# Hawkeye-FineGrained/Hawkeye

Measured on NVIDIA H100. Metric: 448x448 images/sec, BCNN VGG-16 train step (fwd+CE+bwd+grad all-reduce+SGD), device-timed, max over ranks, higher is better.
Workload: dtype tf32 (fp32 storage, fp32 accumulate)

## Files before the change

### hawkeye_b200/csrc/conv.cu

```cuda
#include <stdlib.h>

#include "common.cuh"
#include "host.h"
#include "gemm.h"
#include "../../include/hawkeye_b200.h"

namespace hk {

__global__ void pack_weights_kernel(const float* __restrict__ W, float* __restrict__ Wf, float* __restrict__ Wd,
                                    int Cout, int Cin, int round) {
  const size_t n = (size_t)Cout * Cin * 9;
  for (size_t i = blockIdx.x * (size_t)blockDim.x + threadIdx.x; i < n; i += (size_t)gridDim.x * blockDim.x) {
    const int t = i % 9;
    const int ci = (i / 9) % Cin;
    const int co = i / ((size_t)9 * Cin);
    const float v = round ? tf32_round(W[i]) : W[i];
    if (Wf) Wf[((size_t)t * Cout + co) * Cin + ci] = v;
    if (Wd) Wd[((size_t)(8 - t) * Cin + ci) * Cout + co] = v;
  }
}
__global__ void unpack_wgrad_kernel(const float* __restrict__ dWp, float* __restrict__ dW, int Cout, int Cin, int accumulate) {
  const size_t n = (size_t)Cout * Cin * 9;
  for (size_t i = blockIdx.x * (size_t)blockDim.x + threadIdx.x; i < n; i += (size_t)gridDim.x * blockDim.x) {
    const int t = i % 9;
// ... 813 lines not shown
  a.total_tiles = (int)total_tiles;
  a.per = (int)((total_tiles + ks - 1) / ks);
  const dim3 grid((unsigned)out_tiles, (unsigned)((total_tiles + a.per - 1) / a.per));
  CUtensorMap tmDY, tmX;
  int r;
  if ((r = make_act_map(&tmDY, dy, a.N, a.H, a.W, a.Cout, a.TW, a.TH, a.TN))) return r;
  if ((r = make_act_map(&tmX, x, a.N, a.H, a.W, a.Cin, a.TW + 2, a.TH + 2, a.TN))) return r;
  if (a.TW == 16 && a.TH == 4 && a.TN == 1) return launch_wgrad_tile<16, 4, 1>(tmDY, tmX, a, grid, stream);
  if (a.TW == 8 && a.TH == 8 && a.TN == 1) return launch_wgrad_tile<8, 8, 1>(tmDY, tmX, a, grid, stream);
  if (a.TW == 8 && a.TH == 4 && a.TN == 2) return launch_wgrad_tile<8, 4, 2>(tmDY, tmX, a, grid, stream);
  return set_error(HK_ERR_UNSUPPORTED, "conv3x3_wgrad: pixel tile %dx%dx%d has no kernel", a.TW, a.TH, a.TN);
}

static int conv3x3_wgrad_1x(const float* x, const float* dy, float* dwp, float* db, int N, int H, int W, int Cin, int Cout,
                            cudaStream_t stream, bool zero_dw, bool zero_db);

int conv3x3_wgrad(const float* x, const float* dy, float* dwp, float* db, int N, int H, int W, int Cin, int Cout,
                  cudaStream_t stream, bool zero_db = true) {
  if (!precise()) return conv3x3_wgrad_1x(x, dy, dwp, db, N, H, W, Cin, Cout, stream, true, zero_db);
  HK_REQUIRE(x && dy && dwp, HK_ERR_ARG, "conv3x3_wgrad: null pointer");
  const size_t nx = (size_t)N * H * W * Cin, ny = (size_t)N * H * W * Cout;
  Scratch sx(2 * nx * sizeof(float), stream), sy(2 * ny * sizeof(float), stream);
  HK_REQUIRE(sx.p && sy.p, HK_ERR_DRIVER, "conv3x3_wgrad (precise): cudaMallocAsync of the operand halves failed");
  float *xh = sx.f(), *xl = xh + nx, *yh = sy.f(), *yl = yh + ny;
  int r;
  if ((r = tf32_split(x, xh, xl, nx, stream))) return r;
  if ((r = tf32_split(dy, yh, yl, ny, stream))) return r;
  if ((r = conv3x3_wgrad_1x(xh, yh, dwp, db, N, H, W, Cin, Cout, stream, true, zero_db))) return r;
  if ((r = conv3x3_wgrad_1x(xl, yh, dwp, nullptr, N, H, W, Cin, Cout, stream, false, false))) return r;
  return conv3x3_wgrad_1x(xh, yl, dwp, db, N, H, W, Cin, Cout, stream, false, false);
}

static int conv3x3_wgrad_1x(const float* x, const float* dy, float* dwp, float* db, int N, int H, int W, int Cin, int Cout,
                            cudaStream_t stream, bool zero_dw, bool zero_db) {
  HK_REQUIRE(x && dy && dwp, HK_ERR_ARG, "conv3x3_wgrad: null pointer");
  HK_REQUIRE(Cin % 32 == 0 && Cout % 32 == 0, HK_ERR_UNSUPPORTED, "conv3x3_wgrad: Cin=%d Cout=%d unsupported", Cin, Cout);
  WgradArgs a = {};
  a.dWp = dwp; a.db = db; a.N = N; a.H = H; a.W = W; a.Cin = Cin; a.Cout = Cout;
  pick_wgrad_tile(W, H, &a.TW, &a.TH, &a.TN);
  HK_REQUIRE((a.TH + 2) * (a.TW + 2) * a.TN <= WG_RAW_ROWS, HK_ERR_UNSUPPORTED,
             "conv3x3_wgrad: halo patch too large");
  a.tiles_w = (W + a.TW - 1) / a.TW; a.tiles_h = (H + a.TH - 1) / a.TH; a.tiles_n = (N + a.TN - 1) / a.TN;
  cudaError_t e = cudaSuccess;
  if (zero_dw) {
    e = cudaMemsetAsync(dwp, 0, (size_t)9 * Cout * Cin * sizeof(float), stream);
    if (e != cudaSuccess) return set_error((int)e, "cudaMemsetAsync(dWp): %s", cudaGetErrorString(e));
  }
  if (db && zero_db) {
    e = cudaMemsetAsync(db, 0, (size_t)Cout * sizeof(float), stream);
    if (e != cudaSuccess) return set_error((int)e, "cudaMemsetAsync(db): %s", cudaGetErrorString(e));
  }
  return launch_wgrad(x, dy, a, stream);
}

__global__ void im2col_first_kernel(const float* __restrict__ x, float* __restrict__ x27, int N, int H, int W, int round) {
  const long long total = (long long)N * H * W;
  for (long long pix = blockIdx.x * (long long)blockDim.x + threadIdx.x; pix < total;
       pix += (long long)gridDim.x * blockDim.x) {
    const int wq = (int)(pix % W), hq = (int)((pix / W) % H), n = (int)(pix / ((long long)W * H));
    float v[32];
#pragma unroll
    for (int ci = 0; ci < 3; ++ci)
#pragma unroll
      for (int kh = 0; kh < 3; ++kh)
#pragma unroll
        for (int kw = 0; kw < 3; ++kw) {
          const int hh = hq + kh - 1, ww = wq + kw - 1;
          float t = (hh >= 0 && hh < H && ww >= 0 && ww < W) ? __ldg(x + (((size_t)n * 3 + ci) * H + hh) * W + ww) : 0.f;
          v[ci * 9 + kh * 3 + kw] = round ? tf32_round(t) : t;
        }
    v[27] = 1.f; v[28] = v[29] = v[30] = v[31] = 0.f;
    float4* dst = reinterpret_cast<float4*>(x27 + (size_t)pix * 32);
#pragma unroll
    for (int j = 0; j < 8; ++j) dst[j] = make_float4(v[4 * j], v[4 * j + 1], v[4 * j + 2], v[4 * j + 3]);
  }
}
__global__ void pack_first_weights_kernel(const float* __restrict__ w, const float* __restrict__ bias,
                                          float* __restrict__ w27, int Cout, int round) {
  const int i = blockIdx.x * blockDim.x + threadIdx.x;
  if (i >= Cout * 32) return;
  const int co = i / 32, r = i % 32;
  const float t = r < 27 ? w[co * 27 + r] : (r == 27 && bias ? bias[co] : 0.f);
  w27[i] = round ? tf32_round(t) : t;
}

__global__ void maxpool2x2_fwd_kernel(const float* __restrict__ x, float* __restrict__ y, int N, int H, int W, int C,
                                      int out_nchw) {
  const int Ho = H / 2, Wo = W / 2, C4 = C / 4;
  const size_t total = (size_t)N * Ho * Wo * C4;
  for (size_t i = blockIdx.x * (size_t)blockDim.x + threadIdx.x; i < total; i += (size_t)gridDim.x * blockDim.x) {
    const int c4 = i % C4;
    size_t p = i / C4;
    const int wo = p % Wo; p /= Wo;
    const int ho = p % Ho;
    const int n = p / Ho;
    const float4* base = reinterpret_cast<const float4*>(x + (((size_t)n * H + 2 * ho) * W + 2 * wo) * C) + c4;
    const float4 a = base[0], b = base[C4], c = base[(size_t)W * C4], d = base[(size_t)W * C4 + C4];
    float4 m;
    m.x = fmaxf(fmaxf(a.x, b.x), fmaxf(c.x, d.x));
    m.y = fmaxf(fmaxf(a.y, b.y), fmaxf(c.y, d.y));
    m.z = fmaxf(fmaxf(a.z, b.z), fmaxf(c.z, d.z));
    m.w = fmaxf(fmaxf(a.w, b.w), fmaxf(c.w, d.w));
    if (!out_nchw) {
      reinterpret_cast<float4*>(y + (((size_t)n * Ho + ho) * Wo + wo) * C)[c4] = m;
    } else {
      const size_t hw = (size_t)Ho * Wo, o = ((size_t)n * C + c4 * 4) * hw + (size_t)ho * Wo + wo;
      y[o] = m.x; y[o + hw] = m.y; y[o + 2 * hw] = m.z; y[o + 3 * hw] = m.w;
    }
  }
}

__global__ void maxpool2x2_bwd_kernel(const float* __restrict__ x, const float* __restrict__ dy,
                                      float* __restrict__ dx, int N, int H, int W, int C, int dy_nchw) {
  const int Ho = H / 2, Wo = W / 2;
  const size_t total = (size_t)N * Ho * Wo * C;
  for (size_t i = blockIdx.x * (size_t)blockDim.x + threadIdx.x; i < total; i += (size_t)gridDim.x * blockDim.x) {
    const int c = i % C;
    size_t p = i / C;
    const int wo = p % Wo; p /= Wo;
    const int ho = p % Ho;
    const int n = p / Ho;
    const size_t b00 = (((size_t)n * H + 2 * ho) * W + 2 * wo) * C + c;
    const size_t b01 = b00 + C, b10 = b00 + (size_t)W * C, b11 = b10 + C;
    const float v00 = x[b00], v01 = x[b01], v10 = x[b10], v11 = x[b11];
    const float g = dy_nchw ? dy[((size_t)n * C + c) * Ho * Wo + (size_t)ho * Wo + wo] : dy[i];
    int arg = 0;
    float m = v00;
    if (v01 > m) { m = v01; arg = 1; }
    if (v10 > m) { m = v10; arg = 2; }
    if (v11 > m) { m = v11; arg = 3; }
    const float gm = m > 0.f ? g : 0.f;
    dx[b00] = arg == 0 ? gm : 0.f;
    dx[b01] = arg == 1 ? gm : 0.f;
    dx[b10] = arg == 2 ? gm : 0.f;
    dx[b11] = arg == 3 ? gm : 0.f;
  }
}

__global__ void maxpool2x2_fwd_idx_kernel(const float* __restrict__ x, float* __restrict__ y, unsigned char* __restrict__ code,
                                          int N, int H, int W, int C, int out_nchw) {
  const int Ho = H / 2, Wo = W / 2, C4 = C / 4;
  const size_t total = (size_t)N * Ho * Wo * C4;
  for (size_t i = blockIdx.x * (size_t)blockDim.x + threadIdx.x; i < total; i += (size_t)gridDim.x * blockDim.x) {
    const int c4 = i % C4;
    size_t p = i / C4;
    const int wo = p % Wo; p /= Wo;
    const int ho = p % Ho;
    const int n = p / Ho;
    const float4* base = reinterpret_cast<const float4*>(x + (((size_t)n * H + 2 * ho) * W + 2 * wo) * C) + c4;
    const float4 v0 = base[0], v1 = base[C4], v2 = base[(size_t)W * C4], v3 = base[(size_t)W * C4 + C4];
    float4 m = v0;
    uchar4 a = make_uchar4(0, 0, 0, 0);
#define HK_POOL_STEP(V, K)                     \
    if (V.x > m.x) { m.x = V.x; a.x = K; }     \
    if (V.y > m.y) { m.y = V.y; a.y = K; }     \
    if (V.z > m.z) { m.z = V.z; a.z = K; }     \
    if (V.w > m.w) { m.w = V.w; a.w = K; }
    HK_POOL_STEP(v1, 1) HK_POOL_STEP(v2, 2) HK_POOL_STEP(v3, 3)
#undef HK_POOL_STEP
    a.x |= m.x > 0.f ? 4 : 0; a.y |= m.y > 0.f ? 4 : 0; a.z |= m.z > 0.f ? 4 : 0; a.w |= m.w > 0.f ? 4 : 0;
    reinterpret_cast<uchar4*>(code)[i] = a;
    if (!out_nchw) {
      reinterpret_cast<float4*>(y + (((size_t)n * Ho + ho) * Wo + wo) * C)[c4] = m;
    } else {
      const size_t hw = (size_t)Ho * Wo, o = ((size_t)n * C + c4 * 4) * hw + (size_t)ho * Wo + wo;
      y[o] = m.x; y[o + hw] = m.y; y[o + 2 * hw] = m.z; y[o + 3 * hw] = m.w;
// ... 79 lines not shown
int hk_conv3x3_dgrad(const float* dy, const float* w_dgrad_packed, const float* relu_mask_act, float* dx, int N, int H,
                     int W, int Cin, int Cout, void* stream) {
  return conv3x3_igemm(dy, w_dgrad_packed, nullptr, relu_mask_act, dx, N, H, W, Cout, Cin, 0, (cudaStream_t)stream);
}

size_t hk_conv3x3_wgrad_workspace_bytes(int Cin, int Cout) { return (size_t)9 * Cin * Cout * sizeof(float); }

int hk_conv3x3_wgrad_acc(const float* x, const float* dy, float* dw, float* db, int N, int H, int W, int Cin, int Cout,
                         void* workspace, size_t workspace_bytes, int accumulate, void* stream_) {
  cudaStream_t stream = (cudaStream_t)stream_;
  HK_REQUIRE(workspace && workspace_bytes >= hk_conv3x3_wgrad_workspace_bytes(Cin, Cout), HK_ERR_WORKSPACE,
             "hk_conv3x3_wgrad: workspace too small");
  HK_REQUIRE(dw, HK_ERR_ARG, "hk_conv3x3_wgrad: null dw");
  float* dwp = static_cast<float*>(workspace);
  int r = conv3x3_wgrad(x, dy, dwp, db, N, H, W, Cin, Cout, stream, !accumulate);
  if (r) return r;
  unpack_wgrad_kernel<<<grid_1d((size_t)Cout * Cin * 9, 256), 256, 0, stream>>>(dwp, dw, Cout, Cin, accumulate ? 1 : 0);
  HK_LAUNCH_CHECK("unpack_wgrad_kernel");
  return 0;
}

int hk_conv3x3_wgrad(const float* x, const float* dy, float* dw, float* db, int N, int H, int W, int Cin, int Cout,
                     void* workspace, size_t workspace_bytes, void* stream_) {
  return hk_conv3x3_wgrad_acc(x, dy, dw, db, N, H, W, Cin, Cout, workspace, workspace_bytes, 0, stream_);
}

size_t hk_conv3x3_first_fwd_workspace_bytes(int N, int H, int W, int Cout) {
  return ((size_t)N * H * W * 32 + (size_t)Cout * 32) * sizeof(float);
}

int hk_conv3x3_first_fwd(const float* x_nchw, const float* w, const float* bias, float* y_nhwc, int N, int H, int W,
                         int Cout, void* workspace, size_t workspace_bytes, void* stream_) {
  cudaStream_t stream = (cudaStream_t)stream_;
  HK_REQUIRE(x_nchw && w && y_nhwc, HK_ERR_ARG, "hk_conv3x3_first_fwd: null pointer");
  HK_REQUIRE(Cout % 4 == 0 && Cout <= 256, HK_ERR_UNSUPPORTED, "hk_conv3x3_first_fwd: Cout=%d unsupported", Cout);
  HK_REQUIRE(workspace && workspace_bytes >= hk_conv3x3_first_fwd_workspace_bytes(N, H, W, Cout), HK_ERR_WORKSPACE,
             "hk_conv3x3_first_fwd: workspace too small");
  const long long P = (long long)N * H * W;
  HK_REQUIRE(P < (1ll << 31), HK_ERR_UNSUPPORTED, "hk_conv3x3_first_fwd: too many pixels");
  float* x27 = static_cast<float*>(workspace);
  float* w27 = x27 + (size_t)P * 32;
  const int round = precise() ? 0 : 1;
  im2col_first_kernel<<<grid_1d((size_t)P, 128), 128, 0, stream>>>(x_nchw, x27, N, H, W, round);
  HK_LAUNCH_CHECK("im2col_first_kernel");
  pack_first_weights_kernel<<<(Cout * 32 + 127) / 128, 128, 0, stream>>>(w, bias, w27, Cout, round);
  HK_LAUNCH_CHECK("pack_first_weights_kernel");
  GemmEpi e = {};
  e.C = y_nhwc; e.ldc = Cout; e.alpha = 1.f;
  e.relu = 3;
  return gemm_tf32(x27, 0, 32, 0, w27, 0, 32, 0, e, (int)P, Cout, 32, 1, stream);
}

static int first_wgrad_splits(long long P) {
  for (int S = 592; S > 1; --S)
    if (P % S == 0) return S;
  return 1;
}

size_t hk_conv3x3_first_wgrad_workspace_bytes(int N, int H, int W, int Cout) {
  return (size_t)first_wgrad_splits((long long)N * H * W) * Cout * 32 * sizeof(float);
}

int hk_conv3x3_first_wgrad_acc(const float* x27, const float* dy_nhwc, float* dw, float* db, int N, int H, int W, int Cout,
                               void* workspace, size_t workspace_bytes, int accumulate, void* stream_);
int hk_conv3x3_first_wgrad(const float* x27, const float* dy_nhwc, float* dw, float* db, int N, int H, int W,
                           int Cout, void* workspace, size_t workspace_bytes, void* stream_) {
  return hk_conv3x3_first_wgrad_acc(x27, dy_nhwc, dw, db, N, H, W, Cout, workspace, workspace_bytes, 0, stream_);
}
int hk_conv3x3_first_wgrad_acc(const float* x27, const float* dy_nhwc, float* dw, float* db, int N, int H, int W, int Cout,
                               void* workspace, size_t workspace_bytes, int accumulate, void* stream_) {
  cudaStream_t stream = (cudaStream_t)stream_;
  HK_REQUIRE(x27 && dy_nhwc && dw, HK_ERR_ARG, "hk_conv3x3_first_wgrad: null pointer");
  HK_REQUIRE(Cout % 4 == 0 && Cout <= 128, HK_ERR_UNSUPPORTED, "hk_conv3x3_first_wgrad: Cout=%d unsupported", Cout);
  HK_REQUIRE(workspace && workspace_bytes >= hk_conv3x3_first_wgrad_workspace_bytes(N, H, W, Cout), HK_ERR_WORKSPACE,
             "hk_conv3x3_first_wgrad: workspace too small");
  const long long P = (long long)N * H * W;
  const int S = first_wgrad_splits(P);
  float* part = static_cast<float*>(workspace);
  int r = gemm_splitk(dy_nhwc, 1, Cout, x27, 1, 32, Cout, 32, P, S, part, dw, 27, 27, nullptr, accumulate, stream);
  if (r || !db) return r;
  return sum_splits(part + 27, S, (long long)Cout * 32, Cout, 1, 32, db, 1, nullptr, accumulate, stream);
}

int hk_maxpool2x2_fwd(const float* x_nhwc, float* y, int N, int H, int W, int C, int out_nchw, void* stream) {
  HK_REQUIRE(x_nhwc && y, HK_ERR_ARG, "hk_maxpool2x2_fwd: null pointer");
  HK_REQUIRE(C % 4 == 0 && H % 2 == 0 && W % 2 == 0, HK_ERR_UNSUPPORTED, "hk_maxpool2x2_fwd: C%%4, even H/W required");
  const size_t total = (size_t)N * (H / 2) * (W / 2) * (C / 4);
  maxpool2x2_fwd_kernel<<<grid_1d(total, 256), 256, 0, (cudaStream_t)stream>>>(x_nhwc, y, N, H, W, C, out_nchw);
  HK_LAUNCH_CHECK("maxpool2x2_fwd_kernel");
  return 0;
}

int hk_maxpool2x2_bwd(const float* x_nhwc, const float* dy, float* dx_nhwc, int N, int H, int W, int C, int dy_nchw,
                      void* stream) {
  HK_REQUIRE(x_nhwc && dy && dx_nhwc, HK_ERR_ARG, "hk_maxpool2x2_bwd: null pointer");
  HK_REQUIRE(H % 2 == 0 && W % 2 == 0, HK_ERR_UNSUPPORTED, "hk_maxpool2x2_bwd: even H/W required");
  const size_t total = (size_t)N * (H / 2) * (W / 2) * C;
  maxpool2x2_bwd_kernel<<<grid_1d(total, 256), 256, 0, (cudaStream_t)stream>>>(x_nhwc, dy, dx_nhwc, N, H, W, C, dy_nchw);
  HK_LAUNCH_CHECK("maxpool2x2_bwd_kernel");
  return 0;
}

int hk_maxpool2x2_fwd_idx(const float* x_nhwc, float* y, unsigned char* code, int N, int H, int W, int C, int out_nchw,
                          void* stream) {
  HK_REQUIRE(x_nhwc && y && code, HK_ERR_ARG, "hk_maxpool2x2_fwd_idx: null pointer");
  HK_REQUIRE(C % 4 == 0 && H % 2 == 0 && W % 2 == 0, HK_ERR_UNSUPPORTED, "hk_maxpool2x2_fwd_idx: C%%4, even H/W required");
  const size_t total = (size_t)N * (H / 2) * (W / 2) * (C / 4);
  maxpool2x2_fwd_idx_kernel<<<grid_1d(total, 256), 256, 0, (cudaStream_t)stream>>>(x_nhwc, y, code, N, H, W, C, out_nchw);
  HK_LAUNCH_CHECK("maxpool2x2_fwd_idx_kernel");
  return 0;
}

int hk_maxpool2x2_bwd_idx(const unsigned char* code, const float* dy, float* dx_nhwc, int N, int H, int W, int C,
                          int dy_nchw, void* stream) {
  HK_REQUIRE(code && dy && dx_nhwc, HK_ERR_ARG, "hk_maxpool2x2_bwd_idx: null pointer");
  HK_REQUIRE(C % 4 == 0 && H % 2 == 0 && W % 2 == 0, HK_ERR_UNSUPPORTED, "hk_maxpool2x2_bwd_idx: C%%4, even H/W required");
  const size_t total = (size_t)N * (H / 2) * (W / 2) * (C / 4);
  maxpool2x2_bwd_idx_kernel<<<grid_1d(total, 256), 256, 0, (cudaStream_t)stream>>>(code, dy, dx_nhwc, N, H, W, C, dy_nchw);
  HK_LAUNCH_CHECK("maxpool2x2_bwd_idx_kernel");
  return 0;
}

}
```

### hawkeye_b200/ops.py

```python
import torch
from torch.autograd import Function

from . import _lib

CAPTURE = None


def _grad_ready(p):
    g = getattr(p, 'grad', None)
    return (g is not None and p.requires_grad and g.is_cuda and g.dtype == torch.float32 and g.is_contiguous()
            and g.shape == p.shape and not p._backward_hooks and not getattr(p, '_post_accumulate_grad_hooks', None))


def _check_cuda(*ts):
    for t in ts:
        if t is not None and not t.is_cuda:
            raise _lib.HawkeyeLibError('hawkeye_b200 ops need CUDA tensors (there is no CPU fallback)')


def _f32c(t):
    if t.dtype != torch.float32:
        raise _lib.HawkeyeLibError(f'hawkeye_b200 ops are fp32 (got {t.dtype})')
    return t.contiguous()

# ... 298 lines not shown
            _lib.call('hk_linear_wgrad', dy, x, dw, db, B, F, N, s)
        return dx, dw, db


def linear(x, w, b):
    return LinearFn.apply(x, w, b)


def check_num_classes(n):
    if int(n) % 4 != 0:
        raise _lib.HawkeyeLibError(f'num_classes={n}: hawkeye_b200 classifiers need num_classes % 4 == 0 (16-byte TMA row '
                                   'pitch of the logit gradients); pad the label space to the next multiple of 4')


class CrossEntropyLSFn(Function):
    @staticmethod
    def forward(ctx, logits, labels, smoothing):
        _check_cuda(logits, labels)
        logits = _f32c(logits)
        labels = labels.contiguous().to(torch.int64)
        B, K = logits.shape
        loss = torch.empty(1, device=logits.device, dtype=torch.float32)
        dlogits = torch.empty_like(logits)
        correct = torch.empty(1, device=logits.device, dtype=torch.int32)
        _lib.call('hk_softmax_ce_ls', logits, labels, loss, dlogits, correct, B, K, float(smoothing), 1.0,
                  _lib.stream_ptr())
        ctx.save_for_backward(dlogits)
        ctx.mark_non_differentiable(correct)
        return loss[0], correct

    @staticmethod
    def backward(ctx, g, _g_correct=None):
        (dlogits,) = ctx.saved_tensors
        return dlogits * g, None, None


class CrossEntropyLS(torch.nn.Module):

    def __init__(self, label_smoothing=0.1):
        super().__init__()
        self.label_smoothing = label_smoothing

    def forward(self, logits, labels):
        loss, correct = CrossEntropyLSFn.apply(logits, labels, self.label_smoothing)
        self.last_correct = correct
        return loss


def _vgg_layers(cfg):
    layers = []
    for v in cfg:
        if v != 'M':
            layers.append((int(v), False))
        elif layers and not layers[-1][1]:
            layers[-1] = (layers[-1][0], True)
        else:
            raise _lib.HawkeyeLibError('VGG cfg: every max-pool must follow a conv')
    if not layers[-1][1]:
        raise _lib.HawkeyeLibError('VGG cfg must end with a max-pool (reference BCNN keeps the last pool)')
    return layers


class VGGFeaturesFn(Function):

    @staticmethod
    def forward(ctx, x, cfg, save, *params):
        _check_cuda(x, *params)
        x = _f32c(x)
        s = _lib.stream_ptr()
        dev = x.device
        N, cin0, H, W = x.shape
        if cin0 != 3:
            raise _lib.HawkeyeLibError('VGG features expect a 3-channel NCHW image')
        layers = _vgg_layers(cfg)
        records = []
        cur, C = x, 3
        fuse_ok = not _lib.get_precise() and CAPTURE is None
        for li, (cout, pool) in enumerate(layers):
            w, b = _f32c(params[2 * li]), params[2 * li + 1]
            rec = dict(inp=cur, H=H, W=W)
            fused = pool and li > 0 and fuse_ok and H % 2 == 0 and W % 2 == 0
            if li == 0:
                y = torch.empty(N, H, W, cout, device=dev, dtype=torch.float32)
                ws0 = _ws(_lib.query('hk_conv3x3_first_fwd_workspace_bytes', N, H, W, cout), dev)
                _lib.call('hk_conv3x3_first_fwd', x, w, b, y, N, H, W, cout, ws0, ws0.numel(), s)
                rec['x27'] = ws0 if save else None
            else:
                wf, rec['wd'] = conv3x3_pack(w, save)
                if not fused:
                    y = conv3x3_fwd(cur, wf, b, relu=True)
            if not fused and CAPTURE is not None:
                CAPTURE.append(('relu', y))
            if pool:
                last = li == len(layers) - 1
                Ho, Wo = H // 2, W // 2
                out = torch.empty((N, cout, Ho, Wo) if last else (N, Ho, Wo, cout), device=dev, dtype=torch.float32)
                code = torch.empty(N, Ho, Wo, cout, device=dev, dtype=torch.uint8) if save else None
                if fused:
                    _lib.call('hk_conv3x3_fwd_pool', cur, wf, b, out, code, N, H, W, C, cout, int(last), s)
                elif save:
                    _lib.call('hk_maxpool2x2_fwd_idx', y, out, code, N, H, W, cout, int(last), s)
                else:
                    _lib.call('hk_maxpool2x2_fwd', y, out, N, H, W, cout, int(last), s)
                if CAPTURE is not None:
                    CAPTURE.append(('pool2', y))
                rec.update(code=code, last=last)
                y, H, W = out, Ho, Wo
            records.append(rec)
            cur, C = y, cout
        ctx.layers, ctx.records, ctx.nparams = layers, (records if save else None), len(params)
        ctx.params = params if save else None
        return cur

    @staticmethod
    def backward(ctx, dfeat):
        if ctx.records is None:
            return (None, None, None) + (None,) * ctx.nparams
        s = _lib.stream_ptr()
        g = _f32c(dfeat)
        grads = [None] * ctx.nparams
        for li in reversed(range(len(ctx.layers))):
            rec, (cout, pool) = ctx.records[li], ctx.layers[li]
            N, H, W = g.shape[0], rec['H'], rec['W']
            if pool:
                dx = torch.empty(N, H, W, cout, device=g.device, dtype=torch.float32)
                _lib.call('hk_maxpool2x2_bwd_idx', rec['code'], g, dx, N, H, W, cout, int(rec['last']), s)
                g = dx
            pw, pb = ctx.params[2 * li], ctx.params[2 * li + 1]
            direct = _grad_ready(pw) and _grad_ready(pb)
            if direct:
                dw, db = pw.grad, pb.grad
            else:
                dw = torch.empty(pw.shape, device=g.device, dtype=torch.float32)
                db = torch.empty(cout, device=g.device, dtype=torch.float32)
                grads[2 * li], grads[2 * li + 1] = dw, db
            if li == 0:
                ws = _ws(_lib.query('hk_conv3x3_first_wgrad_workspace_bytes', N, H, W, cout), g.device)
                _lib.call('hk_conv3x3_first_wgrad_acc', rec['x27'], g, dw, db, N, H, W, cout, ws, ws.numel(), int(direct), s)
            else:
                conv3x3_wgrad(rec['inp'], g, dw, db, accumulate=direct)
                g = conv3x3_dgrad(g, rec['wd'], mask=None if ctx.layers[li - 1][1] else rec['inp'])
        ctx.records = ctx.params = None
        return (None, None, None) + tuple(grads)


def vgg_features(x, cfg, params):
    return VGGFeaturesFn.apply(x, tuple(cfg), wants_grad(x, params), *params)


def gemm_tf32(A, B, a_mn=False, b_mn=False, M=None, N=None, K=None, alpha=1.0, diag=0.0, D=None, beta=0.0,
              alpha_vec=None, beta_vec=None, trans_c=False, relu=False, out=None):
    _check_cuda(A, B)
    A, B = _f32c(A), _f32c(B)
    batch = max(A.shape[0] if A.dim() == 3 else 1, B.shape[0] if B.dim() == 3 else 1)
    a2, b2 = A.shape[-2:], B.shape[-2:]
    M_ = a2[1] if a_mn else a2[0]
    K_ = a2[0] if a_mn else a2[1]
    N_ = b2[1] if b_mn else b2[0]
    M, N, K = M or M_, N or N_, K or K_
    sA = a2[0] * a2[1] if A.dim() == 3 else 0
    sB = b2[0] * b2[1] if B.dim() == 3 else 0
    if out is None:
        out = torch.empty((batch, N, M) if trans_c else (batch, M, N), device=A.device, dtype=torch.float32)
    ldc = out.shape[-1]
    sD = ldd = 0
    if D is not None:
        D = _f32c(D)
        ldd = D.shape[-1] if D.shape[-2] != 1 else 0
        sD = D.shape[-2] * D.shape[-1] if D.dim() == 3 else 0
    gemm(A, a_mn, a2[1], sA, B, b_mn, b2[1], sB, out, ldc, out.shape[-2] * out.shape[-1], M, N, K, batch, alpha, alpha_vec,
         diag, D, ldd, sD, beta, beta_vec, relu, trans_c)
    return out


def count_sketch_hashes(input_dim, output_dim):
    import numpy as np
    h1 = np.random.RandomState(1).randint(output_dim, size=input_dim)
    s1 = 2 * np.random.RandomState(3).randint(2, size=input_dim) - 1
    h2 = np.random.RandomState(5).randint(output_dim, size=input_dim)
    s2 = 2 * np.random.RandomState(7).randint(2, size=input_dim) - 1
    return h1.astype(np.int64), s1.astype(np.int64), h2.astype(np.int64), s2.astype(np.int64)


class CompactBilinearPoolFn(Function):
    @staticmethod
    def forward(ctx, x, h1, h2, s1, s2, d):
        _check_cuda(x, h1, h2, s1, s2)
        x = _f32c(x)
        B, C, H, W = x.shape
        y = torch.empty(B, d, device=x.device, dtype=torch.float32)
        pre = torch.empty(B, d, device=x.device, dtype=torch.float32)
        _lib.call('hk_cbp_fwd', x, h1, h2, s1, s2, y, pre, B, C, H * W, d, _lib.stream_ptr())
        if CAPTURE is not None:
            CAPTURE.append(('ssqrt', pre))
        ctx.save_for_backward(x, pre, h1, h2, s1, s2)
        ctx.d = d
        return y

    @staticmethod
    def backward(ctx, dy):
        x, pre, h1, h2, s1, s2 = ctx.saved_tensors
        B, C, H, W = x.shape
        d = ctx.d
        dx = torch.empty_like(x)
        ws = _ws(_lib.query('hk_cbp_bwd_workspace_bytes', B, C, d), x.device)
        _lib.call('hk_cbp_bwd', x, pre, _f32c(dy), h1, h2, s1, s2, dx, B, C, H * W, d, ws, ws.numel(),
                  _lib.stream_ptr())
        return dx, None, None, None, None, None


class CovpoolFn(Function):

    @staticmethod
    def forward(ctx, x):
        _check_cuda(x)
        x = _f32c(x)
        B, C, H, W = x.shape
        cov = torch.empty(B, C, C, device=x.device, dtype=torch.float32)
        xc = torch.empty(B, C, (H * W + 3) // 4 * 4, device=x.device, dtype=torch.float32)
# ... 70 lines not shown
```

### include/hawkeye_b200.h

```cpp
#ifndef HAWKEYE_B200_H
#define HAWKEYE_B200_H
#include <stddef.h>
#include <stdint.h>

#ifdef __cplusplus
extern "C" {
#endif

const char* hk_version(void);
const char* hk_last_error(void);
long long hk_launch_count(void);
void hk_reset_launch_count(void);

void hk_set_precise(int on);
int hk_get_precise(void);

int hk_gemm_tf32(const float* A, int a_mn_major, long long lda, long long strideA, const float* B, int b_mn_major,
                 long long ldb, long long strideB, float* C, long long ldc, long long strideC, int trans_c, int M,
                 int N, int K, int batch, float alpha, const float* alpha_vec, float diag, const float* D,
                 long long ldd, long long strideD, float beta, const float* beta_vec, int relu, void* stream);

int hk_gemm_3xtf32(const float* A, int a_mn_major, long long lda, long long strideA, const float* B, int b_mn_major,
                   long long ldb, long long strideB, float* C, long long ldc, long long strideC, int trans_c, int M,
                   int N, int K, int batch, float alpha, const float* alpha_vec, float diag, const float* D,
                   long long ldd, long long strideD, float beta, const float* beta_vec, int relu, void* stream);

size_t hk_bilinear_pool_fwd_workspace_bytes(int B, int C, int HW);
int hk_bilinear_pool_fwd(const float* x, float* y, float* inv_norm_out, int B, int C, int HW, void* workspace,
                         size_t workspace_bytes, void* stream);
size_t hk_bilinear_pool_bwd_workspace_bytes(int B, int C, int HW);
int hk_bilinear_pool_bwd(const float* x, const float* dy, float* dx, int B, int C, int HW, void* workspace,
                         size_t workspace_bytes, void* stream);

int hk_cbp_fwd(const float* x, const int* h1, const int* h2, const float* s1, const float* s2, float* y, float* pre,
               int B, int C, int HW, int d, void* stream);
size_t hk_cbp_bwd_workspace_bytes(int B, int C, int d);
int hk_cbp_bwd(const float* x, const float* pre, const float* dy, const int* h1, const int* h2, const float* s1,
               const float* s2, float* dx, int B, int C, int HW, int d, void* workspace, size_t workspace_bytes,
               void* stream);

int hk_covpool_fwd(const float* x, float* cov, float* xc, int B, int C, int M, void* stream);
int hk_covpool_bwd(const float* xc, const float* g, float* dx, int B, int C, int M, void* stream);
size_t hk_sqrtm_saved_floats(int B, int n, int iterN);
size_t hk_sqrtm_fwd_workspace_bytes(int B, int n);
size_t hk_sqrtm_bwd_workspace_bytes(int B, int n);
int hk_sqrtm_fwd(const float* x, float* y, float* saved, int B, int n, int iterN, void* workspace,
                 size_t workspace_bytes, void* stream);
int hk_sqrtm_bwd(const float* x, const float* y, const float* g, float* saved, float* grad_x, int B, int n, int iterN,
                 void* workspace, size_t workspace_bytes, void* stream);
int hk_triuvec_fwd(const float* x, float* y, int B, int n, void* stream);
int hk_triuvec_bwd(const float* g, float* dx, int B, int n, void* stream);

int hk_conv3x3_pack_weights(const float* w, float* w_fwd, float* w_dgrad, int Cout, int Cin, void* stream);
int hk_conv3x3_fwd(const float* x_nhwc, const float* w_fwd_packed, const float* bias, float* y_nhwc, int N, int H,
                   int W, int Cin, int Cout, int relu, void* stream);
int hk_conv3x3_fwd_pool(const float* x_nhwc, const float* w_fwd_packed, const float* bias, float* pooled,
                        unsigned char* code, int N, int H, int W, int Cin, int Cout, int out_nchw, void* stream);
int hk_conv3x3_s2_fwd(const float* x_nhwc, const float* w_fwd_packed, const float* bias, float* y_nhwc, int N, int H,
                      int W, int Cin, int Cout, int relu, void* stream);
int hk_conv3x3_dgrad(const float* dy_nhwc, const float* w_dgrad_packed, const float* relu_mask_act, float* dx_nhwc,
                     int N, int H, int W, int Cin, int Cout, void* stream);
size_t hk_conv3x3_wgrad_workspace_bytes(int Cin, int Cout);
int hk_conv3x3_wgrad(const float* x_nhwc, const float* dy_nhwc, float* dw, float* db, int N, int H, int W, int Cin,
                     int Cout, void* workspace, size_t workspace_bytes, void* stream);
int hk_conv3x3_wgrad_acc(const float* x_nhwc, const float* dy_nhwc, float* dw, float* db, int N, int H, int W, int Cin,
                         int Cout, void* workspace, size_t workspace_bytes, int accumulate, void* stream);
size_t hk_conv3x3_first_fwd_workspace_bytes(int N, int H, int W, int Cout);
int hk_conv3x3_first_fwd(const float* x_nchw, const float* w, const float* bias, float* y_nhwc, int N, int H, int W,
                         int Cout, void* workspace, size_t workspace_bytes, void* stream);
size_t hk_conv3x3_first_wgrad_workspace_bytes(int N, int H, int W, int Cout);
int hk_conv3x3_first_wgrad(const float* x27, const float* dy_nhwc, float* dw, float* db, int N, int H, int W,
                           int Cout, void* workspace, size_t workspace_bytes, void* stream);
int hk_conv3x3_first_wgrad_acc(const float* x27, const float* dy_nhwc, float* dw, float* db, int N, int H, int W,
                               int Cout, void* workspace, size_t workspace_bytes, int accumulate, void* stream);
int hk_maxpool2x2_fwd(const float* x_nhwc, float* y, int N, int H, int W, int C, int out_nchw, void* stream);
int hk_maxpool2x2_bwd(const float* x_nhwc, const float* dy, float* dx_nhwc, int N, int H, int W, int C, int dy_nchw,
                      void* stream);
int hk_maxpool2x2_fwd_idx(const float* x_nhwc, float* y, unsigned char* code, int N, int H, int W, int C, int out_nchw,
                          void* stream);
int hk_maxpool2x2_bwd_idx(const unsigned char* code, const float* dy, float* dx_nhwc, int N, int H, int W, int C,
                          int dy_nchw, void* stream);

int hk_stem_im2col(const float* x_nchw, float* x147, int N, int H, int W, void* stream);
int hk_pack_stem_weights(const float* w, float* w147, int Cout, void* stream);
size_t hk_bn_workspace_bytes(long long P, int C);
int hk_bn_fwd(const float* x, const float* gamma, const float* beta, const float* residual, float* y, float* save_mean,
              float* save_invstd, float* running_mean, float* running_var, float momentum, float eps, long long P, int C,
              int relu, void* workspace, size_t workspace_bytes, void* stream);
int hk_bn_apply(const float* x, const float* mean, const float* invstd, const float* gamma, const float* beta,
                const float* residual, float* y, long long P, int C, int relu, void* stream);
int hk_bn_bwd(const float* x, const float* y, const float* dy, const float* gamma, const float* save_mean,
              const float* save_invstd, float* dx, float* dres, float* dgamma, float* dbeta, long long P, int C, int relu,
              void* workspace, size_t workspace_bytes, void* stream);
int hk_bn_bwd_ex(const float* x, const float* y, const float* dy, const float* gamma, const float* beta_for_mask,
                 const float* save_mean, const float* save_invstd, float* dx, float* dres, float* dgamma, float* dbeta,
                 long long P, int C, int relu, void* workspace, size_t workspace_bytes, void* stream);
int hk_bn_bwd_frozen(const float* x, const float* y, const float* dy, const float* gamma, const float* beta_for_mask,
                     const float* mean, const float* invstd, float* dx, float* dres, float* dgamma, float* dbeta, long long P,
                     int C, int relu, void* workspace, size_t workspace_bytes, void* stream);
int hk_maxpool3x3s2_fwd(const float* x, float* y, unsigned char* argmax, int N, int H, int W, int C, void* stream);
int hk_maxpool3x3s2_bwd(const unsigned char* argmax, const float* dy, float* dx, int N, int H, int W, int C,
                        void* stream);
int hk_subsample2(const float* x, float* y, int N, int H, int W, int C, void* stream);
int hk_upsample2_zero(const float* y, float* x, int N, int H, int W, int C, void* stream);
int hk_add_inplace(float* a, const float* b, size_t n, void* stream);
int hk_nhwc_to_nchw(const float* x, float* y, int N, int HW, int C, void* stream);
int hk_nchw_to_nhwc(const float* x, float* y, int N, int HW, int C, void* stream);
int hk_act_fwd(const float* x, float* y, size_t n, int elu, void* stream);
int hk_act_bwd(const float* y, const float* dy, float* dx, size_t n, int elu, void* stream);
size_t hk_matconv_wgrad_workspace_bytes(long long P, int K, int Cout);
int hk_matconv_wgrad(const float* x, const float* dy, float* dw, long long P, int K, int Cout, void* workspace,
                     size_t workspace_bytes, void* stream);

int hk_softmax_neg_rows_fwd(const float* g, float* w, long long rows, int cols, void* stream);
int hk_softmax_neg_rows_bwd(const float* w, const float* dw, float* dg, long long rows, int cols, void* stream);
int hk_cci_weight_fwd(const float* w_sci, const float* weight, float* w_cci, int B, long long per, void* stream);
int hk_cci_weight_bwd(const float* w_sci, const float* weight, const float* d_cci, float* d_sci, float* d_weight, int B,
                      long long per, void* stream);
int hk_row_mean_fwd(const float* x, float* y, long long rows, int cols, int ld, void* stream);
int hk_row_mean_bwd(const float* dy, float* dx, long long rows, int cols, int ld, void* stream);
int hk_cin_pair_diff_fwd(const float* z, float* d, int B, long long per, void* stream);
int hk_cin_pair_diff_bwd(const float* dd, float* dz, int B, long long per, void* stream);
int hk_cin_contrastive_loss(const float* p, const long long* labels, float* loss, float* dp, int B, int R, float alpha,
                            void* stream);

int hk_se_gate_fwd(const float* x, const float* m, float* s, long long rows, int hw, void* stream);
int hk_se_gate_bwd(const float* x, const float* m, const float* ds, float* dx, float* dm, long long rows, int hw,
                   void* stream);
int hk_l2norm_rows_fwd(const float* x, float* y, float* inv_norm, int rows, int D, void* stream);
int hk_l2norm_rows_bwd(const float* y, const float* inv_norm, const float* dy, float* dx, int rows, int D, void* stream);
int hk_npair_loss(const float* prod, const int* cls, const int* part, double* loss_acc, float* dprod, int n, void* stream);

int hk_apinet_pairs(const float* pool, const long long* labels, long long* intra, long long* inter, long long* labels1,
                    long long* labels2, int n, int D, void* stream);
int hk_apinet_gather(const float* pool, const long long* idx2, float* mutual, int n, int D, void* stream);
int hk_apinet_scatter(const float* dmutual, const long long* idx2, float* dpool, int n, int D, void* stream);
int hk_dropout_fwd(const float* x, float* y, size_t n, float p, const long long* seed, int call, void* stream);
int hk_dropout_bwd(const float* dy, float* dx, size_t n, float p, const long long* seed, int call, void* stream);
int hk_apinet_gate_fwd(const float* m, const float* mutual, float* out, int rows, int D, float p, const long long* seed,
                       int call0, void* stream);
int hk_apinet_gate_bwd(const float* m, const float* mutual, const float* dout, float* dm, float* dmutual, int rows, int D,
                       float p, const long long* seed, int call0, void* stream);
int hk_apinet_rank_loss(const float* logits, const long long* targets, double* loss_acc, float* dlogits, int R, int K,
                        float margin, float grad_scale, void* stream);

size_t hk_dcl_head_workspace_bytes(int N, int C, int H, int W);
int hk_dcl_head_fwd(const float* x, const float* w, const float* b, float* pooled, float* mask, int N, int C, int H, int W,
                    void* workspace, size_t workspace_bytes, void* stream);
int hk_dcl_head_bwd(const float* x, const float* w, const float* mask, const float* dpooled, const float* dmask, float* dx,
                    float* dw, float* db, int N, int C, int H, int W, void* workspace, size_t workspace_bytes, void* stream);
int hk_dcl_loss(const float* logits, int ld, int K, int K2, const long long* labels, const long long* labels_swap,
                const float* mask, const float* law, int R, int Q, float alpha, float beta, float gamma, int combine,
                double* loss_acc, float* dlogits, float* dmask, int* correct, void* stream);

int hk_prototree_dist_fwd(const float* x, const float* protos, float* z, float* mind, int* argmin, int N, int HW, int D,
                          int P, int act, void* stream);
int hk_prototree_dist_bwd(const float* z, const float* protos, const float* mind, const int* argmin, const float* dmind,
// ... 127 lines not shown
```

Measured before the change: 698.9.

## Fuse im2col into first-layer conv forward and weight-gradient WGMMA kernels

Result: faster. 742.3, median of 6 (+6.2%).

```diff
diff --git a/hawkeye_b200/csrc/conv.cu b/hawkeye_b200/csrc/conv.cu
--- a/hawkeye_b200/csrc/conv.cu
+++ b/hawkeye_b200/csrc/conv.cu
@@ -919,6 +919,149 @@
   const int co = i / 32, r = i % 32;
   const float t = r < 27 ? w[co * 27 + r] : (r == 27 && bias ? bias[co] : 0.f);
   w27[i] = round ? tf32_round(t) : t;
+}
+
+__device__ __forceinline__ float x27_value(const float* __restrict__ x, int n, int hq, int wq, int j, int H, int W) {
+  if (j >= 27) return j == 27 ? 1.f : 0.f;
+  const int ci = j / 9, hh = hq + (j % 9) / 3 - 1, ww = wq + j % 3 - 1;
+  return (hh >= 0 && hh < H && ww >= 0 && ww < W) ? tf32_round(__ldg(x + (((size_t)n * 3 + ci) * H + hh) * W + ww)) : 0.f;
+}
+
+constexpr int FIRST_FWD_PIX = 128;
+constexpr int FIRST_FWD_SMEM = 1024 + FIRST_FWD_PIX * 128 + 64 * 128;
+__global__ void __launch_bounds__(128) first_fwd_direct_kernel(const float* __restrict__ x, const float* __restrict__ w,
+                                                               const float* __restrict__ bias, float* __restrict__ y,
+                                                               int N, int H, int W) {
+  extern __shared__ uint8_t smem_raw[];
+  uint8_t* sA = reinterpret_cast<uint8_t*>((reinterpret_cast<uintptr_t>(smem_raw) + 1023) & ~uintptr_t(1023));
+  uint8_t* sB = sA + FIRST_FWD_PIX * 128;
+  const int t = threadIdx.x;
+  const long long P = (long long)N * H * W, p0 = (long long)blockIdx.x * FIRST_FWD_PIX;
+  {
+    const long long p = p0 + t;
+    float v[32];
+    if (p < P) {
+      const int wq = (int)(p % W), hq = (int)((p / W) % H), n = (int)(p / ((long long)W * H));
+#pragma unroll
+      for (int j = 0; j < 32; ++j) v[j] = x27_value(x, n, hq, wq, j, H, W);
+    } else {
+#pragma unroll
+      for (int j = 0; j < 32; ++j) v[j] = 0.f;
+    }
+#pragma unroll
+    for (int j = 0; j < 32; j += 4)
+      *reinterpret_cast<float4*>(sA + sw128_off(t, j)) = make_float4(v[j], v[j + 1], v[j + 2], v[j + 3]);
+    const int co = t >> 1, c0 = (t & 1) * 16;
+#pragma unroll
+    for (int j = 0; j < 16; j += 4) {
+      float4 q;
+      float* qq = reinterpret_cast<float*>(&q);
+#pragma unroll
+      for (int e = 0; e < 4; ++e) {
+        const int r = c0 + j + e;
+        qq[e] = tf32_round(r < 27 ? __ldg(w + co * 27 + r) : (r == 27 && bias ? __ldg(bias + co) : 0.f));
+      }
+      *reinterpret_cast<float4*>(sB + sw128_off(co, c0 + j)) = q;
+    }
+  }
+  fence_proxy_async();
+  __syncthreads();
+  const uint64_t b_base = make_sdesc(smem_u32(sB));
+  float acc[2][32];
+#pragma unroll
+  for (int m = 0; m < 2; ++m)
+#pragma unroll
+    for (int i = 0; i < 32; ++i) acc[m][i] = 0.f;
+  wgmma_fence();
+#pragma unroll
+  for (int m = 0; m < 2; ++m) {
+    const uint64_t a_base = make_sdesc(smem_u32(sA + m * 64 * 128));
+#pragma unroll
+    for (int ks = 0; ks < 4; ++ks) wgmma_tf32(acc[m], a_base + ks * 2, b_base + ks * 2, 1);
+  }
+  wgmma_commit();
+  wgmma_wait<0>();
+  wgmma_keep(acc[0]);
+  wgmma_keep(acc[1]);
+  const int warp = t >> 5, lane = t & 31;
+#pragma unroll
+  for (int m = 0; m < 2; ++m)
+#pragma unroll
+    for (int h = 0; h < 2; ++h) {
+      const long long p = p0 + m * 64 + warp * 16 + (lane >> 2) + 8 * h;
+      if (p >= P) continue;
+      float* dst = y + p * 64 + 2 * (lane & 3);
+#pragma unroll
+      for (int i = 0; i < 8; ++i)
+        *reinterpret_cast<float2*>(dst + 8 * i) =
+            make_float2(tf32_round(fmaxf(acc[m][4 * i + 2 * h], 0.f)), tf32_round(fmaxf(acc[m][4 * i + 2 * h + 1], 0.f)));
+    }
+}
+
+constexpr int FIRST_WG_THREADS = 256;
+constexpr int FIRST_WG_SMEM = 1024 + 64 * 33 * 4;
+__global__ void __launch_bounds__(FIRST_WG_THREADS, 2) first_wgrad_direct_kernel(const float* __restrict__ x,
+                                                                              const float* __restrict__ dy,
+                                                                              float* __restrict__ part, int N, int H, int W) {
+  extern __shared__ uint8_t smem_raw[];
+  uint8_t* smem = reinterpret_cast<uint8_t*>((reinterpret_cast<uintptr_t>(smem_raw) + 1023) & ~uintptr_t(1023));
+  const int wg = threadIdx.x >> 7, t = threadIdx.x & 127, warp = t >> 5, lane = t & 31;
+  uint8_t* sB = smem + wg * 32 * 128;
+  const int P = N * H * W, nblk = (P + 31) / 32;
+  const uint64_t b_base = make_sdesc(smem_u32(sB));
+  float acc[16];
+#pragma unroll
+  for (int i = 0; i < 16; ++i) acc[i] = 0.f;
+  const int co = warp * 16 + (lane >> 2);
+  for (int blk = blockIdx.x * 2 + wg; blk < nblk; blk += gridDim.x * 2) {
+    const int pb = blk * 32;
+    uint32_t a[4][4];
+#pragma unroll
+    for (int ks = 0; ks < 4; ++ks)
+#pragma unroll
+      for (int e = 0; e < 4; ++e) {
+        const int p = pb + 8 * ks + (lane & 3) + 4 * (e >> 1);
+        a[ks][e] = p < P ? __float_as_uint(__ldg(dy + (size_t)p * 64 + co + 8 * (e & 1))) : 0u;
+      }
+    float v[8];
+    {
+      const int p = pb + lane;
+      if (p < P) {
+        const int wq = p % W, hq = (p / W) % H, n = p / (W * H);
+#pragma unroll
+        for (int jj = 0; jj < 8; ++jj) v[jj] = x27_value(x, n, hq, wq, warp * 8 + jj, H, W);
+      } else {
+#pragma unroll
+        for (int jj = 0; jj < 8; ++jj) v[jj] = 0.f;
+      }
+    }
+    named_bar(1 + wg, 128);
+#pragma unroll
+    for (int jj = 0; jj < 8; ++jj) *reinterpret_cast<float*>(sB + sw128_off(warp * 8 + jj, lane)) = v[jj];
+    fence_proxy_async();
+    named_bar(1 + wg, 128);
+    wgmma_fence();
+#pragma unroll
+    for (int ks = 0; ks < 4; ++ks) wgmma_tf32(acc, a[ks], b_base + ks * 2);
+    wgmma_commit();
+    wgmma_wait<0>();
+    wgmma_keep(acc);
+  }
+  __syncthreads();
+  float* red = reinterpret_cast<float*>(smem);
+  if (wg == 1) {
+#pragma unroll
+    for (int i = 0; i < 16; ++i) red[(co + 8 * ((i >> 1) & 1)) * 33 + 8 * (i >> 2) + 2 * (lane & 3) + (i & 1)] = acc[i];
+  }
+  __syncthreads();
+  if (wg == 0) {
+    float* dst = part + (size_t)blockIdx.x * 64 * 32;
+#pragma unroll
+    for (int i = 0; i < 16; ++i) {
+      const int r = co + 8 * ((i >> 1) & 1), c = 8 * (i >> 2) + 2 * (lane & 3) + (i & 1);
+      dst[r * 32 + c] = acc[i] + red[r * 33 + c];
+    }
+  }
 }
 
 __global__ void maxpool2x2_fwd_kernel(const float* __restrict__ x, float* __restrict__ y, int N, int H, int W, int C,
@@ -1164,6 +1307,46 @@
   return sum_splits(part + 27, S, (long long)Cout * 32, Cout, 1, 32, db, 1, nullptr, accumulate, stream);
 }
 
+int hk_conv3x3_first_fwd_direct(const float* x_nchw, const float* w, const float* bias, float* y_nhwc, int N, int H, int W,
+                                int Cout, void* stream) {
+  HK_REQUIRE(!precise(), HK_ERR_UNSUPPORTED, "hk_conv3x3_first_fwd_direct: not available in 3xTF32 mode");
+  HK_REQUIRE(x_nchw && w && y_nhwc, HK_ERR_ARG, "hk_conv3x3_first_fwd_direct: null pointer");
+  HK_REQUIRE(Cout == 64, HK_ERR_UNSUPPORTED, "hk_conv3x3_first_fwd_direct: Cout=%d unsupported (64 only)", Cout);
+  HK_REQUIRE(N > 0 && H > 0 && W > 0, HK_ERR_ARG, "hk_conv3x3_first_fwd_direct: empty map");
+  HK_REQUIRE((reinterpret_cast<uintptr_t>(y_nhwc) & 7) == 0, HK_ERR_ALIGN, "hk_conv3x3_first_fwd_direct: y not 8-byte aligned");
+  const long long P = (long long)N * H * W;
+  HK_REQUIRE(P < (1ll << 31), HK_ERR_UNSUPPORTED, "hk_conv3x3_first_fwd_direct: too many pixels");
+  first_fwd_direct_kernel<<<(int)((P + FIRST_FWD_PIX - 1) / FIRST_FWD_PIX), 128, FIRST_FWD_SMEM, (cudaStream_t)stream>>>(
+      x_nchw, w, bias, y_nhwc, N, H, W);
+  HK_LAUNCH_CHECK("first_fwd_direct_kernel");
+  return 0;
+}
+
+static int first_wgrad_direct_ctas() { return 2 * num_sms(); }
+
+size_t hk_conv3x3_first_wgrad_direct_workspace_bytes(void) {
+  return (size_t)first_wgrad_direct_ctas() * 64 * 32 * sizeof(float);
+}
+
+int hk_conv3x3_first_wgrad_direct_acc(const float* x_nchw, const float* dy_nhwc, float* dw, float* db, int N, int H, int W,
+                                      int Cout, void* workspace, size_t workspace_bytes, int accumulate, void* stream_) {
+  cudaStream_t stream = (cudaStream_t)stream_;
+  HK_REQUIRE(!precise(), HK_ERR_UNSUPPORTED, "hk_conv3x3_first_wgrad_direct: not available in 3xTF32 mode");
+  HK_REQUIRE(x_nchw && dy_nhwc && dw, HK_ERR_ARG, "hk_conv3x3_first_wgrad_direct: null pointer");
+  HK_REQUIRE(Cout == 64, HK_ERR_UNSUPPORTED, "hk_conv3x3_first_wgrad_direct: Cout=%d unsupported (64 only)", Cout);
+  HK_REQUIRE(N > 0 && H > 0 && W > 0, HK_ERR_ARG, "hk_conv3x3_first_wgrad_direct: empty map");
+  HK_REQUIRE(workspace && workspace_bytes >= hk_conv3x3_first_wgrad_direct_workspace_bytes(), HK_ERR_WORKSPACE,
+             "hk_conv3x3_first_wgrad_direct: workspace too small");
+  HK_REQUIRE((long long)N * H * W < (1ll << 31), HK_ERR_UNSUPPORTED, "hk_conv3x3_first_wgrad_direct: too many pixels");
+  const int G = first_wgrad_direct_ctas();
+  float* part = static_cast<float*>(workspace);
+  first_wgrad_direct_kernel<<<G, FIRST_WG_THREADS, FIRST_WG_SMEM, stream>>>(x_nchw, dy_nhwc, part, N, H, W);
+  HK_LAUNCH_CHECK("first_wgrad_direct_kernel");
+  int r = sum_splits(part, G, 64 * 32, 64, 27, 32, dw, 27, nullptr, accumulate, stream);
+  if (r || !db) return r;
+  return sum_splits(part + 27, G, 64 * 32, 64, 1, 32, db, 1, nullptr, accumulate, stream);
+}
+
 int hk_maxpool2x2_fwd(const float* x_nhwc, float* y, int N, int H, int W, int C, int out_nchw, void* stream) {
   HK_REQUIRE(x_nhwc && y, HK_ERR_ARG, "hk_maxpool2x2_fwd: null pointer");
   HK_REQUIRE(C % 4 == 0 && H % 2 == 0 && W % 2 == 0, HK_ERR_UNSUPPORTED, "hk_maxpool2x2_fwd: C%%4, even H/W required");
diff --git a/hawkeye_b200/ops.py b/hawkeye_b200/ops.py
--- a/hawkeye_b200/ops.py
+++ b/hawkeye_b200/ops.py
@@ -404,9 +404,13 @@
             fused = pool and li > 0 and fuse_ok and H % 2 == 0 and W % 2 == 0
             if li == 0:
                 y = torch.empty(N, H, W, cout, device=dev, dtype=torch.float32)
-                ws0 = _ws(_lib.query('hk_conv3x3_first_fwd_workspace_bytes', N, H, W, cout), dev)
-                _lib.call('hk_conv3x3_first_fwd', x, w, b, y, N, H, W, cout, ws0, ws0.numel(), s)
-                rec['x27'] = ws0 if save else None
+                rec['direct'] = fuse_ok and cout == 64
+                if rec['direct']:
+                    _lib.call('hk_conv3x3_first_fwd_direct', x, w, b, y, N, H, W, cout, s)
+                else:
+                    ws0 = _ws(_lib.query('hk_conv3x3_first_fwd_workspace_bytes', N, H, W, cout), dev)
+                    _lib.call('hk_conv3x3_first_fwd', x, w, b, y, N, H, W, cout, ws0, ws0.numel(), s)
+                    rec['x27'] = ws0 if save else None
             else:
                 wf, rec['wd'] = conv3x3_pack(w, save)
                 if not fused:
@@ -456,7 +460,11 @@
                 dw = torch.empty(pw.shape, device=g.device, dtype=torch.float32)
                 db = torch.empty(cout, device=g.device, dtype=torch.float32)
                 grads[2 * li], grads[2 * li + 1] = dw, db
-            if li == 0:
+            if li == 0 and rec['direct']:
+                ws = _ws(_lib.query('hk_conv3x3_first_wgrad_direct_workspace_bytes'), g.device)
+                _lib.call('hk_conv3x3_first_wgrad_direct_acc', rec['inp'], g, dw, db, N, H, W, cout, ws, ws.numel(),
+                          int(direct), s)
+            elif li == 0:
                 ws = _ws(_lib.query('hk_conv3x3_first_wgrad_workspace_bytes', N, H, W, cout), g.device)
                 _lib.call('hk_conv3x3_first_wgrad_acc', rec['x27'], g, dw, db, N, H, W, cout, ws, ws.numel(), int(direct), s)
             else:
diff --git a/include/hawkeye_b200.h b/include/hawkeye_b200.h
--- a/include/hawkeye_b200.h
+++ b/include/hawkeye_b200.h
@@ -73,6 +73,11 @@
                            int Cout, void* workspace, size_t workspace_bytes, void* stream);
 int hk_conv3x3_first_wgrad_acc(const float* x27, const float* dy_nhwc, float* dw, float* db, int N, int H, int W,
                                int Cout, void* workspace, size_t workspace_bytes, int accumulate, void* stream);
+int hk_conv3x3_first_fwd_direct(const float* x_nchw, const float* w, const float* bias, float* y_nhwc, int N, int H, int W,
+                                int Cout, void* stream);
+size_t hk_conv3x3_first_wgrad_direct_workspace_bytes(void);
+int hk_conv3x3_first_wgrad_direct_acc(const float* x_nchw, const float* dy_nhwc, float* dw, float* db, int N, int H, int W,
+                                      int Cout, void* workspace, size_t workspace_bytes, int accumulate, void* stream);
 int hk_maxpool2x2_fwd(const float* x_nhwc, float* y, int N, int H, int W, int C, int out_nchw, void* stream);
 int hk_maxpool2x2_bwd(const float* x_nhwc, const float* dy, float* dx_nhwc, int N, int H, int W, int C, int dy_nchw,
                       void* stream);
```
